# nvlong21/Lightweight-face-detection-CenterNet

Hardware: AMD Instinct MI355X
Metric: images/sec at 640x640 batch inference (higher is better)
Workload: dtype bf16; 1 GPU; BASELINE configs[1]: batch=64 640x640 bf16 on 1 MI355X per rank, forward + top-100 peak decode; synthetic uint8 images resident in HBM, calibrated synthetic weights (seed 0); 2 context(s) per GPU, batch k on context k mod 2; batch_per_gpu=64, global_batch=64, topk=100, parallelism=dp1, contexts_per_gpu=2, input_buffers=4

## Files before the change

### lightweight-face-detection-centernet_amd/csrc/cf_mbconv3.hip

```cpp
#include "cf_exp.h"
#include "cf_common.h"
#include "cf_kernels.h"
#include "cf_mx.h"
#include <cstdlib>

namespace cf {

template <int KS, int JX, int TOH, int TOW, int NW, bool ALDS = true>
struct Mx {
    static constexpr int HC = 32;
    static constexpr int IH = TOH + KS - 1, IWQ = TOW / 4 + 1, IWP = IWQ * 4;
    static constexpr int NQD = IH * IWQ, NIB = (NQD + 7) / 8, IPX = NQD * 4;
    static constexpr int CP = HC * 8 + 16;
    static constexpr int EBYTES = NIB * 8 * CP;
    static constexpr int NOQ = TOH * (TOW / 4), NSET = (NOQ + 15) / 16;
    static constexpr int WXB = JX * 1024;
    static constexpr int NSTEP = KS * 2;
    static constexpr int ATB = 2 * NSTEP * 512;
    static constexpr int LDS = EBYTES + WXB + (ALDS ? ATB : 0);
    static_assert(TOW % 4 == 0 && KS <= 5, "x-quads; two k-steps cover 4 + KS - 1 <= 8 inputs");
};

template <int KS, int JX, int TOH, int TOW, int NW, bool ALDS>
__global__ __launch_bounds__(NW * 64) void expdw_mx_kernel(MbParams p) {
    typedef Mx<KS, JX, TOH, TOW, NW, ALDS> G;
    constexpr int IWQ = G::IWQ, IWP = G::IWP, IPX = G::IPX, NIB = G::NIB, CP = G::CP, NSET = G::NSET, WXB = G::WXB;
    extern __shared__ __attribute__((aligned(16))) char smem[];
    char* E = smem;
    char* Wst = smem + G::EBYTES;

    const int tid = threadIdx.x, lane = tid & 63;
    const int wave = __builtin_amdgcn_readfirstlane(tid >> 6);
    const int pl = lane & 31, h = lane >> 5;
    const int tiles_x = (p.Wout + TOW - 1) / TOW;
    const int tyi = blockIdx.x / tiles_x, txi = blockIdx.x - tyi * tiles_x;
    const int ox0 = txi * TOW, oy0 = tyi * TOH, b = blockIdx.z;
    const int grp = blockIdx.y;

    {
        const char* srcx = (const char*)p.wexp + (size_t)grp * WXB;
        for (int c = wave; c < WXB / 1024; c += NW)
            __builtin_amdgcn_global_load_lds((const __attribute__((address_space(1))) void*)(srcx + c * 1024 + lane * 16),
                                             (__attribute__((address_space(3))) void*)(Wst + c * 1024), 16, 0, 0);
    }
    asm volatile("" ::: "memory");
    char* Ats = Wst + WXB;
    u32x2 A[ALDS ? 1 : 2][ALDS ? 1 : KS][2];
    if constexpr (ALDS) {
        const char* srca = (const char*)p.wdw + (size_t)grp * G::ATB;
        for (int c = wave; c < G::ATB / 1024; c += NW)
            __builtin_amdgcn_global_load_lds((const __attribute__((address_space(1))) void*)(srca + c * 1024 + lane * 16),
                                             (__attribute__((address_space(3))) void*)(Ats + c * 1024), 16, 0, 0);
    } else {
        const u32x2* at = reinterpret_cast<const u32x2*>(p.wdw) + (size_t)grp * (2 * KS * 2) * 64 + lane;
#pragma unroll
        for (int q = 0; q < 2; ++q)
#pragma unroll
            for (int ky = 0; ky < KS; ++ky)
#pragma unroll
                for (int ks = 0; ks < 2; ++ks) A[q][ky][ks] = at[((q * KS + ky) * 2 + ks) * 64];
    }
    asm volatile("" ::: "memory");
    const char* xbase = (const char*)p.x + (size_t)b * p.Hin * p.Win * p.Cin * 2;
    const unsigned rowbytes = (unsigned)p.Cin * 2;
    auto load_x = [&](int ib, u32x4* xf) -> bool {
        const int ip = ib * 32 + pl;
        const int ipc = ip < IPX ? ip : IPX - 1;
        const int iy = ipc / IWP, ix = ipc - iy * IWP;
        const int gy = oy0 - p.pad_lo + iy, gx = ox0 - p.pad_lo + ix;
        const int cy = min(max(gy, 0), p.Hin - 1), cx = min(max(gx, 0), p.Win - 1);
        if (p.xblock) {
            const char* xb = (const char*)p.x + blk_off(((size_t)b * p.Hin + cy) * p.Win + cx, p.Cin / 8, h * JX);
#pragma unroll
            for (int j = 0; j < JX; ++j) xf[j] = ld16(xb + j * 512);
        } else {
            const unsigned off = ((unsigned)cy * (unsigned)p.Win + (unsigned)cx) * rowbytes + (unsigned)(h * JX * 16);
#pragma unroll
            for (int j = 0; j < JX; ++j) xf[j] = ld16(xbase + off + j * 16);
        }
        return ip < IPX && (unsigned)gy < (unsigned)p.Hin && (unsigned)gx < (unsigned)p.Win;
    };
    const bool last_in = (h * JX + JX - 1) * 8 < p.Cin;
    auto mask_x = [&](u32x4* xf, bool valid) {
#pragma unroll
        for (int j = 0; j < JX; ++j) {
            const bool vj = j == JX - 1 ? (valid && last_in) : valid;
            xf[j].x = vj ? xf[j].x : 0u; xf[j].y = vj ? xf[j].y : 0u; xf[j].z = vj ? xf[j].z : 0u; xf[j].w = vj ? xf[j].w : 0u;
        }
    };
#ifdef CF_ABLATION
    const int abl = p.nw;
#else
    constexpr int abl = 0;
#endif
    u32x4 xa[JX];
    bool va = false;
    if (wave < NIB) va = load_x(wave, xa);
    static_assert(NIB >= NW, "every wave issues the X loads the wait below keeps in flight");
    cf_sync_lds_dma_keep<(ALDS ? 0 : 2 * KS * 2) + JX>();
    mask_x(xa, va);

    for (int ib = wave; ib < NIB; ib += NW) {
        u32x4 xn[JX];
        const bool more = ib + NW < NIB;
        bool vn = false;
        if (more) { if (abl & 8) { for (int j = 0; j < JX; ++j) xn[j] = xa[j]; vn = va; } else vn = load_x(ib + NW, xn); }
        f32x16 a;
#pragma unroll
        for (int r = 0; r < 16; ++r) a[r] = 0.0f;
        const char* wb = Wst + lane * 16;
#pragma unroll
        for (int j = 0; j < JX; ++j) {
            const u32x4 wv = ld16(wb + j * 1024);
            a = __builtin_amdgcn_mfma_f32_32x32x16_bf16(__builtin_bit_cast(mfma_bf16x8, xa[j]),
                                                        __builtin_bit_cast(mfma_bf16x8, wv), a, 0, 0, 0);
        }
        char* ecell = E + (unsigned)(ib * 8 + h) * (unsigned)CP + pl * 8;
#pragma unroll
        for (int t = 0; t < 4; ++t) {
            f32x2 u0, u1; u0.x = a[4 * t]; u0.y = a[4 * t + 1]; u1.x = a[4 * t + 2]; u1.y = a[4 * t + 3];
            f32x2 y0 = u0, y1 = u1;
            if (!(abl & 4)) { y0 = swish2_pre(u0); y1 = swish2_pre(u1); }
            u32x2 d;
            d.x = __builtin_bit_cast(uint32_t, __builtin_amdgcn_cvt_pkrtz(y0.x, y0.y));
            d.y = __builtin_bit_cast(uint32_t, __builtin_amdgcn_cvt_pkrtz(y1.x, y1.y));
            *reinterpret_cast<u32x2*>(ecell + 2 * t * CP) = d;
        }
        if (more) {
#pragma unroll
            for (int j = 0; j < JX; ++j) xa[j] = xn[j];
            mask_x(xa, vn);
        }
    }
    __syncthreads();

    static constexpr SetMap<TOH, TOW, IWQ> kSets{};
    const int kg = lane >> 4;
    for (int set = wave; set < NSET; set += NW) {
        const uint32_t e = kSets.v[set * 16 + (lane & 15)];
        const int oy = (e >> 6) & 0x1ff, oxq = e & 63;
        const bool live = (e & 0x8000u) == 0;
        f32x4 acc[8];
        const char* bb = E + (unsigned)(oy * IWQ + oxq) * (unsigned)CP + kg * 64;
        if (abl & 1) {
#pragma unroll
            for (int g = 0; g < 8; ++g) acc[g] = f32x4{(float)oy, (float)oxq, (float)g, 1.0f};
        } else {
        if constexpr (ALDS) mx_depthwise_lds<KS, IWQ, CP>(bb, Ats + lane * 8, acc);
        else mx_depthwise<KS, IWQ, CP>(bb, reinterpret_cast<const u32x2 (*)[KS][2]>(A), acc);
        }
        if (!(abl & 2))
#pragma unroll
        for (int g = 0; g < 8; ++g)
#pragma unroll
            for (int i = 0; i < 4; i += 2) {
                f32x2 u; u.x = acc[g][i]; u.y = acc[g][i + 1];
                const f32x2 y = swish2_pre(u) * kNegLn23;
                acc[g][i] = y.x; acc[g][i + 1] = y.y;
            }
        const int gy = oy0 + oy, gx0 = ox0 + 4 * oxq;
        if (!live || gy >= p.Hout || ((abl & 16) && acc[0][0] != 123.0f)) continue;
        const size_t opix0 = ((size_t)b * p.Hout + gy) * p.Wout + gx0;
        const int chunk = grp * 4 + kg;
#pragma unroll
        for (int i = 0; i < 4; ++i) {
            if (gx0 + i >= p.Wout) break;
            u32x4 o;
            o.x = packb(acc[0][i], acc[1][i]); o.y = packb(acc[2][i], acc[3][i]);
            o.z = packb(acc[4][i], acc[5][i]); o.w = packb(acc[6][i], acc[7][i]);
            const size_t opix = opix0 + i;
            if (abl & 32) {
                const size_t region = (((size_t)b * gridDim.x + blockIdx.x) * gridDim.y + grp) * (size_t)(TOH * TOW * 64);
                st16((char*)p.y + region + ((size_t)((set * 4 + i) * 1024 + lane * 16)) % (size_t)(TOH * TOW * 64), o);
                continue;
            }
            st16((char*)p.y + (p.yblock ? blk_off(opix, p.hid / 8, chunk) : (opix * p.hid + (size_t)chunk * 8) * 2), o);
        }
    }
}

#include CF_EXP_INC(cf_mbconv3_0)

template <int KS, int JX, int NMB, int TOH, int TOW, int NW, bool TAIL16, bool ALDS = false>
struct Fx {
    static constexpr int IH = TOH + KS - 1, IWQ = TOW / 4 + 1, IWP = IWQ * 4;
    static constexpr int NQD = IH * IWQ, NIB = (NQD + 7) / 8, IPX = NQD * 4, MAXI = (NIB + NW - 1) / NW;
    static constexpr int CP8 = 32 * 8 + 16, CP4 = 16 * 8 + 16;
    static constexpr int EBYTES = NIB * 8 * CP8;
    static constexpr int NOQ = TOH * (TOW / 4), NSET = (NOQ + 15) / 16, SPW = NSET / NW;
    static constexpr int WXB = JX * 1024;
    static constexpr int ATB = 2 * KS * 2 * 512;
    static constexpr int LDS = EBYTES + 2 * WXB + (ALDS ? ATB : 0);
    static_assert(NSET % NW == 0, "every wave owns SPW whole sets (project accumulators live in registers)");
    static_assert(TOW % 4 == 0 && KS <= 5 && (NMB == 2 || NMB == 4 || NMB == 6), "geometry");
    static_assert(!TAIL16 || JX <= 2, "16-channel round: one 16x16x32 expand MFMA, Cin <= 32");
};

template <int KS, int JX, int NMB, bool RESID, int TOH, int TOW, int NW, bool TAIL16, bool XRELOAD, bool ALDS, bool SB = false>
__global__ __launch_bounds__(NW * 64) void mbconv_mx_kernel(MbParams p) {
    typedef Fx<KS, JX, NMB, TOH, TOW, NW, TAIL16, ALDS> G;
    constexpr int IWQ = G::IWQ, IWP = G::IWP, IPX = G::IPX, NIB = G::NIB, MAXI = G::MAXI, CP8 = G::CP8, CP4 = G::CP4;
    constexpr int SPW = G::SPW, WXB = G::WXB;
    extern __shared__ __attribute__((aligned(16))) char smem[];
    char* E = smem;
    char* Wst = smem + G::EBYTES;
    char* Ats = Wst + 2 * G::WXB;

    const int tid = threadIdx.x, lane = tid & 63;
    const int wave = __builtin_amdgcn_readfirstlane(tid >> 6);
    const int pl = lane & 31, h = lane >> 5, kg = lane >> 4;
    const int ox0 = blockIdx.x * TOW, oy0 = blockIdx.y * TOH, b = blockIdx.z;
    const int nq = p.nq;
#ifdef CF_ABLATION
    const int abl = p.nw;
#else
    constexpr int abl = 0;
#endif

    const char* xbase = (const char*)p.x + (size_t)b * p.Hin * p.Win * p.Cin * 2;
    const unsigned rowbytes = (unsigned)p.Cin * 2;

    auto stage_weights = [&](int q) {
        char* dst = Wst + (q & 1) * WXB;
        const char* srcx = (const char*)p.wexp + (size_t)q * WXB;
        for (int c = wave; c < WXB / 1024; c += NW)
            __builtin_amdgcn_global_load_lds((const __attribute__((address_space(1))) void*)(srcx + c * 1024 + lane * 16),
                                             (__attribute__((address_space(3))) void*)(dst + c * 1024), 16, 0, 0);
    };

    u32x4 xf[MAXI][JX];
    auto load_x = [&]() {
#pragma unroll
    for (int t = 0; t < MAXI; ++t) {
        const int ib = wave + NW * t;
        const int ip = ib * 32 + pl;
        const int ipc = ip < IPX ? ip : IPX - 1;
        const int iy = ipc / IWP, ix = ipc - iy * IWP;
        const int gy = oy0 - p.pad_lo + iy, gx = ox0 - p.pad_lo + ix;
        const bool valid = ip < IPX && (unsigned)gy < (unsigned)p.Hin && (unsigned)gx < (unsigned)p.Win;
        const int cy = min(max(gy, 0), p.Hin - 1), cx = min(max(gx, 0), p.Win - 1);
        const unsigned off = ((unsigned)cy * (unsigned)p.Win + (unsigned)cx) * rowbytes + (unsigned)(h * JX * 16);
#pragma unroll
        for (int j = 0; j < JX; ++j) {
            const bool vj = valid && (h * JX + j) * 8 < p.Cin;
            const u32x4 v = ld16(xbase + off + j * 16);
            xf[t][j].x = vj ? v.x : 0u; xf[t][j].y = vj ? v.y : 0u;
            xf[t][j].z = vj ? v.z : 0u; xf[t][j].w = vj ? v.w : 0u;
        }
    }
    };
    if constexpr (!XRELOAD) load_x();

    static constexpr SetMap<TOH, TOW, IWQ> kSets{};
    unsigned qcell[SPW];
#pragma unroll
    for (int sw = 0; sw < SPW; ++sw) {
        const uint32_t e = kSets.v[(wave * SPW + sw) * 16 + (lane & 15)];
        qcell[sw] = ((e >> 6) & 0x1ff) * IWQ + (e & 63);
    }

    f32x4 pacc[SPW][4][NMB];
#pragma unroll
    for (int sw = 0; sw < SPW; ++sw)
#pragma unroll
        for (int i = 0; i < 4; ++i)
#pragma unroll
            for (int mb = 0; mb < NMB; ++mb) pacc[sw][i][mb] = f32x4{0.0f, 0.0f, 0.0f, 0.0f};

    stage_weights(0);
    asm volatile("" ::: "memory");
    for (int q = 0; q < nq; ++q) {
        const char* wx = Wst + (q & 1) * WXB;
        u32x2 A[ALDS ? 1 : 2][ALDS ? 1 : KS][2];
        if constexpr (!ALDS) {
            const u32x2* at = reinterpret_cast<const u32x2*>(p.wdw) + (size_t)q * (2 * KS * 2) * 64 + lane;
#pragma unroll
            for (int a = 0; a < 2; ++a)
#pragma unroll
                for (int ky = 0; ky < KS; ++ky)
#pragma unroll
                    for (int ks = 0; ks < 2; ++ks) A[a][ky][ks] = at[((a * KS + ky) * 2 + ks) * 64];
        }
        u32x4 wpc[NMB];
#pragma unroll
        for (int mb = 0; mb < NMB; ++mb) wpc[mb] = ld16((const char*)p.wproj + (((size_t)q * NMB + mb) * 64 + lane) * 16);
        if constexpr (XRELOAD) load_x();
        cf_sync_lds_dma_keep<(ALDS ? 0 : 2 * KS * 2) + NMB + (XRELOAD ? MAXI * JX : 0)>();
        if constexpr (ALDS) {
            const char* srca = (const char*)p.wdw + (size_t)q * G::ATB;
            for (int c = wave; c < G::ATB / 1024; c += NW)
                __builtin_amdgcn_global_load_lds((const __attribute__((address_space(1))) void*)(srca + c * 1024 + lane * 16),
                                                 (__attribute__((address_space(3))) void*)(Ats + c * 1024), 16, 0, 0);
        }
        const char* Atq = Ats;

#pragma unroll
        for (int t = 0; t < MAXI; ++t) {
            const int ib = wave + NW * t;
            if (ib >= NIB) break;
            f32x16 a;
#pragma unroll
            for (int r = 0; r < 16; ++r) a[r] = 0.0f;
#pragma unroll
            for (int j = 0; j < JX; ++j) {
                const u32x4 wv = ld16(wx + (j * 64 + lane) * 16);
                a = __builtin_amdgcn_mfma_f32_32x32x16_bf16(__builtin_bit_cast(mfma_bf16x8, xf[t][j]),
                                                            __builtin_bit_cast(mfma_bf16x8, wv), a, 0, 0, 0);
            }
            char* ecell = E + (unsigned)(ib * 8 + h) * (unsigned)CP8 + pl * 8;
#pragma unroll
            for (int tq = 0; tq < 4; ++tq) {
                f32x2 u0, u1; u0.x = a[4 * tq]; u0.y = a[4 * tq + 1]; u1.x = a[4 * tq + 2]; u1.y = a[4 * tq + 3];
                f32x2 y0 = u0, y1 = u1;
                if (!(abl & 4)) { y0 = swish2_pre(u0); y1 = swish2_pre(u1); }
                u32x2 d;
                d.x = __builtin_bit_cast(uint32_t, __builtin_amdgcn_cvt_pkrtz(y0.x, y0.y));
                d.y = __builtin_bit_cast(uint32_t, __builtin_amdgcn_cvt_pkrtz(y1.x, y1.y));
                *reinterpret_cast<u32x2*>(ecell + 2 * tq * CP8) = d;
            }
        }
        cf_sync_lds_dma();
        if (q + 1 < nq) stage_weights(q + 1);
        asm volatile("" ::: "memory");

#pragma unroll
        for (int sw = 0; sw < SPW; ++sw) {
            f32x4 acc[8];
            if (abl & 1) {
#pragma unroll
                for (int g = 0; g < 8; ++g) acc[g] = f32x4{(float)q, (float)g, 1.0f, 2.0f};
            } else {
            if constexpr (ALDS && SB) mx_depthwise_lds1<KS, IWQ, CP8>(E + qcell[sw] * (unsigned)CP8 + kg * 64, Atq + lane * 8, acc);
            else if constexpr (ALDS) mx_depthwise_lds<KS, IWQ, CP8>(E + qcell[sw] * (unsigned)CP8 + kg * 64, Atq + lane * 8, acc);
            else mx_depthwise<KS, IWQ, CP8>(E + qcell[sw] * (unsigned)CP8 + kg * 64, reinterpret_cast<const u32x2 (*)[KS][2]>(A), acc);
            }
            if (!(abl & 2))
#pragma unroll
            for (int g = 0; g < 8; ++g)
#pragma unroll
                for (int i = 0; i < 4; i += 2) {
                    f32x2 u; u.x = acc[g][i]; u.y = acc[g][i + 1];
                    const f32x2 y = swish2_pre(u);
                    acc[g][i] = y.x; acc[g][i + 1] = y.y;
                }
#pragma unroll
            for (int i = 0; i < 4; ++i) {
                u32x4 d;
                d.x = packb(acc[0][i], acc[1][i]); d.y = packb(acc[2][i], acc[3][i]);
                d.z = packb(acc[4][i], acc[5][i]); d.w = packb(acc[6][i], acc[7][i]);
                if (abl & 8) { pacc[sw][i][0][0] += __uint_as_float(d.x ^ d.y ^ d.z ^ d.w); continue; }
#pragma unroll
                for (int mb = 0; mb < NMB; ++mb)
                    pacc[sw][i][mb] = __builtin_amdgcn_mfma_f32_16x16x32_bf16(__builtin_bit_cast(mfma_bf16x8, wpc[mb]),
                                                                             __builtin_bit_cast(mfma_bf16x8, d), pacc[sw][i][mb], 0, 0, 0);
            }
        }
    }

    if constexpr (TAIL16) {
        typedef __attribute__((ext_vector_type(4))) __bf16 mfma_bf16x4;
        const u32x4 wv = ld16((const char*)p.wexp + (size_t)nq * WXB + lane * 16);
        u32x2 A4[KS][2];
        {
            const u32x2* at = reinterpret_cast<const u32x2*>(p.wdw) + (size_t)nq * (2 * KS * 2) * 64 + lane;
#pragma unroll
            for (int ky = 0; ky < KS; ++ky)
#pragma unroll
                for (int ks = 0; ks < 2; ++ks) A4[ky][ks] = at[(ky * 2 + ks) * 64];
        }
        u32x2 wp4[NMB];
#pragma unroll
        for (int mb = 0; mb < NMB; ++mb)
            wp4[mb] = *reinterpret_cast<const u32x2*>((const char*)p.wproj + (size_t)nq * NMB * 1024 + ((size_t)mb * 64 + lane) * 8);
        __syncthreads();
        for (int sb = wave; sb < NIB * 2; sb += NW) {
            const int ip = sb * 16 + (lane & 15), kc = lane >> 4;
            const int ipc = ip < IPX ? ip : IPX - 1;
            const int iy = ipc / IWP, ix = ipc - iy * IWP;
            const int gy = oy0 - p.pad_lo + iy, gx = ox0 - p.pad_lo + ix;
            const bool valid = ip < IPX && (unsigned)gy < (unsigned)p.Hin && (unsigned)gx < (unsigned)p.Win && kc * 8 < p.Cin;
            const int cy = min(max(gy, 0), p.Hin - 1), cx = min(max(gx, 0), p.Win - 1);
            u32x4 xv = ld16(xbase + ((unsigned)cy * (unsigned)p.Win + (unsigned)cx) * rowbytes + (unsigned)(min(kc * 8, p.Cin - 8) * 2));
            xv.x = valid ? xv.x : 0u; xv.y = valid ? xv.y : 0u; xv.z = valid ? xv.z : 0u; xv.w = valid ? xv.w : 0u;
            f32x4 a4 = {0.0f, 0.0f, 0.0f, 0.0f};
            a4 = __builtin_amdgcn_mfma_f32_16x16x32_bf16(__builtin_bit_cast(mfma_bf16x8, xv), __builtin_bit_cast(mfma_bf16x8, wv), a4, 0, 0, 0);
            f32x2 u0, u1; u0.x = a4[0]; u0.y = a4[1]; u1.x = a4[2]; u1.y = a4[3];
            const f32x2 y0 = swish2_pre(u0), y1 = swish2_pre(u1);
            u32x2 d;
            d.x = __builtin_bit_cast(uint32_t, __builtin_amdgcn_cvt_pkrtz(y0.x, y0.y));
            d.y = __builtin_bit_cast(uint32_t, __builtin_amdgcn_cvt_pkrtz(y1.x, y1.y));
            *reinterpret_cast<u32x2*>(E + (unsigned)(sb * 4 + kc) * (unsigned)CP4 + (lane & 15) * 8) = d;
        }
        __syncthreads();
#pragma unroll
        for (int sw = 0; sw < SPW; ++sw) {
            const char* bb = E + qcell[sw] * (unsigned)CP4 + kg * 32;
            f32x4 acc[4];
#pragma unroll
            for (int g = 0; g < 4; ++g) acc[g] = f32x4{0.0f, 0.0f, 0.0f, 0.0f};
#pragma unroll
            for (int st = 0; st < KS * 2; ++st) {
                const char* bs = bb + ((st >> 1) * IWQ + (st & 1)) * CP4;
// ... 646 lines not shown
```

### lightweight-face-detection-centernet_amd/csrc/cf_mx.h

```cpp
#pragma once
#include "cf_common.h"

namespace cf {

typedef __attribute__((ext_vector_type(8))) __bf16 mfma_bf16x8;
typedef __attribute__((ext_vector_type(4))) _Float16 mfma_f16x4;
static constexpr float kNegLog2e3 = -1.44269504088896341f, kNegLn23 = -0.69314718055994531f;

typedef __attribute__((ext_vector_type(2))) __bf16 bf16x2_v;
__device__ __forceinline__ uint32_t packb(float lo, float hi) {
    f32x2 v; v.x = lo; v.y = hi;
    return __builtin_bit_cast(uint32_t, __builtin_convertvector(v, bf16x2_v));
}
__device__ __forceinline__ u32x4 pack16b(const float* f) {
    u32x4 c; c.x = packb(f[0], f[1]); c.y = packb(f[2], f[3]); c.z = packb(f[4], f[5]); c.w = packb(f[6], f[7]); return c;
}

__device__ __forceinline__ f32x2 swish2_pre(f32x2 u) {
    f32x2 e; e.x = __builtin_amdgcn_exp2f(u.x); e.y = __builtin_amdgcn_exp2f(u.y);
    const f32x2 den = e + 1.0f;
    f32x2 r; r.x = __builtin_amdgcn_rcpf(den.x); r.y = __builtin_amdgcn_rcpf(den.y);
    return u * r;
}

static inline uint16_t host_f32_to_f16_3(float f) {
    uint32_t u; __builtin_memcpy(&u, &f, 4);
    const uint32_t sign = (u >> 16) & 0x8000u;
    const int32_t exp = (int32_t)((u >> 23) & 0xff) - 127 + 15;
    uint32_t man = u & 0x7fffffu;
    if (((u >> 23) & 0xff) == 0xff) return (uint16_t)(sign | 0x7c00u | (man ? 0x200u : 0));
    if (exp >= 31) return (uint16_t)(sign | 0x7bffu);
    if (exp <= 0) {
        if (exp < -10) return (uint16_t)sign;
        man |= 0x800000u;
        const int shift = 14 - exp;
        uint32_t half = man >> shift;
        const uint32_t rem = man & ((1u << shift) - 1), mid = 1u << (shift - 1);
        if (rem > mid || (rem == mid && (half & 1))) ++half;
        return (uint16_t)(sign | half);
    }
    uint32_t half = ((uint32_t)exp << 10) | (man >> 13);
    const uint32_t rem = man & 0x1fffu;
    if (rem > 0x1000u || (rem == 0x1000u && (half & 1))) ++half;
    if (half >= 0x7c00u) half = 0x7bffu;
    return (uint16_t)(sign | half);
}

template <int TOH, int TOW, int IWQ, int S = 1>
struct SetMap {
    static constexpr int OWQ = TOW / 4, NOQ = TOH * OWQ, NSET = (NOQ + 15) / 16, NSLOT = NSET * 16;
    static_assert(OWQ <= 64 && TOH <= 256, "entry packing");
    uint16_t v[NSLOT];
    constexpr SetMap() : v() {
        int bucket[16][NOQ] = {}; int cnt[16] = {}, used[16] = {};
        for (int r = 0; r < NOQ; ++r) { const int b = (S * (r / OWQ) * IWQ + (r % OWQ)) & 15; bucket[b][cnt[b]++] = r; }
        int slot[NSLOT] = {};
        for (int s = 0; s < NSET; ++s)
            for (int q = 0; q < 16; ++q) {
                const int b = ((q >> 2) + 4 * (q & 3)) & 15;
                slot[s * 16 + q] = used[b] < cnt[b] ? bucket[b][used[b]++] : -1;
            }
        for (int b = 0; b < 16; ++b)
            while (used[b] < cnt[b]) {
                int s = 0; while (slot[s] >= 0) ++s;
                slot[s] = bucket[b][used[b]++];
            }
        for (int s = 0; s < NSLOT; ++s) {
            const int r = slot[s] >= 0 ? slot[s] : 0;
            v[s] = (uint16_t)((slot[s] < 0 ? 0x8000 : 0) | ((r / OWQ) << 6) | (r % OWQ));
        }
    }
};

#define CF_MX_MFMA(ACC, AV, BV, ABID) ACC = __builtin_amdgcn_mfma_f32_4x4x4f16(AV, BV, ACC, 2, ABID, 0)

template <int KS, int IWQ, int CP>
__device__ __forceinline__ void mx_depthwise(const char* bb, const u32x2 (*A)[KS][2], f32x4* acc) {
    constexpr int NSTEP = KS * 2;
#pragma unroll
    for (int g = 0; g < 8; ++g) acc[g] = f32x4{0.0f, 0.0f, 0.0f, 0.0f};
    u32x4 bq[2][4];
#pragma unroll
    for (int g2 = 0; g2 < 4; ++g2) bq[0][g2] = ld16(bb + g2 * 16);
#pragma unroll
    for (int st = 0; st < NSTEP; ++st) {
        if (st + 1 < NSTEP) {
            const int ky = (st + 1) >> 1, ks = (st + 1) & 1;
#pragma unroll
            for (int g2 = 0; g2 < 4; ++g2) bq[(st + 1) & 1][g2] = ld16(bb + (ky * IWQ + ks) * CP + g2 * 16);
        }
        __builtin_amdgcn_sched_barrier(0);
#pragma unroll
        for (int g = 0; g < 8; ++g) {
            const mfma_f16x4 av = __builtin_bit_cast(mfma_f16x4, A[g >> 2][st >> 1][st & 1]);
            u32x2 b2;
            b2.x = (g & 1) ? bq[st & 1][g >> 1].z : bq[st & 1][g >> 1].x;
            b2.y = (g & 1) ? bq[st & 1][g >> 1].w : bq[st & 1][g >> 1].y;
            const mfma_f16x4 bv = __builtin_bit_cast(mfma_f16x4, b2);
            switch (g & 3) {
                case 0: CF_MX_MFMA(acc[g], av, bv, 0); break;
                case 1: CF_MX_MFMA(acc[g], av, bv, 1); break;
                case 2: CF_MX_MFMA(acc[g], av, bv, 2); break;
                default: CF_MX_MFMA(acc[g], av, bv, 3); break;
            }
        }
        __builtin_amdgcn_sched_barrier(0);
    }
}

template <int KS, int IWQ, int CP>
__device__ __forceinline__ void mx_depthwise_lds(const char* bb, const char* at , f32x4* acc) {
    constexpr int NSTEP = KS * 2;
#pragma unroll
    for (int g = 0; g < 8; ++g) acc[g] = f32x4{0.0f, 0.0f, 0.0f, 0.0f};
    u32x4 bq[2][4];
    u32x2 aq[2][2];
#pragma unroll
    for (int g2 = 0; g2 < 4; ++g2) bq[0][g2] = ld16(bb + g2 * 16);
    aq[0][0] = *reinterpret_cast<const u32x2*>(at);
    aq[0][1] = *reinterpret_cast<const u32x2*>(at + NSTEP * 512);
#pragma unroll
    for (int st = 0; st < NSTEP; ++st) {
        if (st + 1 < NSTEP) {
            const int ky = (st + 1) >> 1, ks = (st + 1) & 1;
#pragma unroll
            for (int g2 = 0; g2 < 4; ++g2) bq[(st + 1) & 1][g2] = ld16(bb + (ky * IWQ + ks) * CP + g2 * 16);
            aq[(st + 1) & 1][0] = *reinterpret_cast<const u32x2*>(at + (st + 1) * 512);
            aq[(st + 1) & 1][1] = *reinterpret_cast<const u32x2*>(at + (NSTEP + st + 1) * 512);
        }
        __builtin_amdgcn_sched_barrier(0);
#pragma unroll
        for (int g = 0; g < 8; ++g) {
            const mfma_f16x4 av = __builtin_bit_cast(mfma_f16x4, aq[st & 1][g >> 2]);
            u32x2 b2;
            b2.x = (g & 1) ? bq[st & 1][g >> 1].z : bq[st & 1][g >> 1].x;
            b2.y = (g & 1) ? bq[st & 1][g >> 1].w : bq[st & 1][g >> 1].y;
            const mfma_f16x4 bv = __builtin_bit_cast(mfma_f16x4, b2);
            switch (g & 3) {
                case 0: CF_MX_MFMA(acc[g], av, bv, 0); break;
                case 1: CF_MX_MFMA(acc[g], av, bv, 1); break;
                case 2: CF_MX_MFMA(acc[g], av, bv, 2); break;
                default: CF_MX_MFMA(acc[g], av, bv, 3); break;
            }
        }
        __builtin_amdgcn_sched_barrier(0);
    }
}

template <int KS, int IWQ, int CP>
__device__ __forceinline__ void mx_depthwise_lds1(const char* bb, const char* at, f32x4* acc) {
    constexpr int NSTEP = KS * 2;
#pragma unroll
    for (int g = 0; g < 8; ++g) acc[g] = f32x4{0.0f, 0.0f, 0.0f, 0.0f};
#pragma unroll
    for (int st = 0; st < NSTEP; ++st) {
        const int ky = st >> 1, ks = st & 1;
// ... 87 lines not shown
```

### lightweight-face-detection-centernet_amd/csrc/cf_stem0.hip

```cpp
#include <type_traits>
#include "cf_common.h"
#include "cf_kernels.h"
#include "cf_mx.h"
#include <vector>
#include "centerface_hip.h"

namespace cf {

typedef __attribute__((ext_vector_type(8))) __bf16 mfma_bf16x8;

static inline int slot_channel(int nb, int i) {
    int h = (i >> 2) & 1;
    int r = (i & 3) + 4 * (i >> 3);
    return nb * 32 + h * 16 + r;
}

constexpr int S0_TOH = 16, S0_TOW = 16;
constexpr int S0_NT = (S0_TOH * S0_TOW / 32) * 64;
constexpr int S0_IH = S0_TOH + 2, S0_IW = S0_TOW + 2, S0_IPX = S0_IH * S0_IW;
constexpr int S0_PH = 2 * S0_IH + 1, S0_PW = 2 * S0_IW + 1;
constexpr int S0_PROW = S0_PW * 3 + 1;

void stem0_lut(float* lut ) {
    const float mean[3] = {0.408f, 0.447f, 0.470f};
// ... 465 lines not shown
                if (decltype(lastb)::value && (tt & 1) + 4 * (tt >> 1) >= VP) continue;
                f32x2 x2; x2.x = a[2 * tt]; x2.y = a[2 * tt + 1];
                const f32x2 y2 = s0_swish2_prescaled(x2);
                *reinterpret_cast<uint32_t*>(ecol + ((tt & 1) + 4 * (tt >> 1)) * S0P_PITCH) =
                    __builtin_bit_cast(uint32_t, __builtin_amdgcn_cvt_pkrtz(y2.x, y2.y));
            }
        };
        if (VP < 16 && t == (S0P_NIB - 1) / S0P_NW && ib == S0P_NIB - 1) activate(std::true_type{});
        else activate(std::false_type{});
    }
    __syncthreads();

    const int par = wave >> 1;
    auto tile_pixel = [](int u, int& oy, int& ox) {
        const int pr = u >> 7, r = u & 127;
        oy = r >> 3; ox = 2 * (r & 7) + pr;
    };
    int dy, dx; tile_pixel((wave * 2 + h) * 32 + pl, dy, dx);
    const char* eb0 = E + (unsigned)((dy * S0_IW + (dx - par)) / 2) * (unsigned)S0P_PITCH;
    const S0_AS4 s0_u32x8* wtab = (const S0_AS4 s0_u32x8*)p.wdw;

    auto dw_chunk = [&](int c) -> u32x4 {
        float a8[8];
        const S0_AS4 s0_u32x8* wq = wtab + ((par * 4 + c) * 3) * 2;
        const char* eb = eb0 + c * 32;
#pragma unroll
        for (int ky = 0; ky < 3; ++ky)
#pragma unroll
            for (int t = 0; t < 2; ++t) {
                const s0_u32x8 wv = wq[ky * 2 + t];
                const char* et = eb + (ky * (S0_IW / 2) + t) * S0P_PITCH;
                const u32x4 e0 = ld16(et), e1 = ld16(et + 16);
                if (ky == 0 && t == 0) { dot8_first(a8, wv, e0, e1); continue; }
                s0_dot2c(a8[0], wv[0], e0.x); s0_dot2c(a8[1], wv[1], e0.y);
                s0_dot2c(a8[2], wv[2], e0.z); s0_dot2c(a8[3], wv[3], e0.w);
                s0_dot2c(a8[4], wv[4], e1.x); s0_dot2c(a8[5], wv[5], e1.y);
                s0_dot2c(a8[6], wv[6], e1.z); s0_dot2c(a8[7], wv[7], e1.w);
            }
#pragma unroll
        for (int i = 0; i < 8; i += 2) {
            f32x2 u; u.x = a8[i]; u.y = a8[i + 1];
            const f32x2 yv = s0_swish2_prescaled(u);
            a8[i] = yv.x; a8[i + 1] = yv.y;
        }
        return pack16<T>(a8);
    };

    f32x16 acc[2];
#pragma unroll
    for (int k = 0; k < 2; ++k)
#pragma unroll
        for (int r = 0; r < 16; ++r) acc[k][r] = 0.0f;
#pragma unroll
    for (int j = 0; j < 2; ++j) {
        const u32x4 wpc = ld16((const char*)p.wproj + ((size_t)j * 64 + lane) * 16);
        const u32x4 dA = dw_chunk(j), dB = dw_chunk(2 + j);
        u32x4 x0, x1;
        {
            auto s0 = __builtin_amdgcn_permlane32_swap(dA.x, dB.x, false, false); x0.x = s0[0]; x1.x = s0[1];
            auto s1 = __builtin_amdgcn_permlane32_swap(dA.y, dB.y, false, false); x0.y = s1[0]; x1.y = s1[1];
            auto s2 = __builtin_amdgcn_permlane32_swap(dA.z, dB.z, false, false); x0.z = s2[0]; x1.z = s2[1];
            auto s3 = __builtin_amdgcn_permlane32_swap(dA.w, dB.w, false, false); x0.w = s3[0]; x1.w = s3[1];
        }
        acc[0] = __builtin_amdgcn_mfma_f32_32x32x16_bf16(__builtin_bit_cast(mfma_bf16x8, wpc), __builtin_bit_cast(mfma_bf16x8, x0), acc[0], 0, 0, 0);
        acc[1] = __builtin_amdgcn_mfma_f32_32x32x16_bf16(__builtin_bit_cast(mfma_bf16x8, wpc), __builtin_bit_cast(mfma_bf16x8, x1), acc[1], 0, 0, 0);
    }
    if (h != 0) return;
#pragma unroll
    for (int k = 0; k < 2; ++k) {
        int oy, ox; tile_pixel((wave * 2 + k) * 32 + pl, oy, ox);
        const int gy = oy0 + oy, gx = ox0 + ox;
        if (gy >= Ho || gx >= Wo) continue;
        T* out = (T*)p.y + (((size_t)b * Ho + gy) * Wo + gx) * 16;
#pragma unroll
        for (int g = 0; g < 2; ++g) {
            float v[8];
#pragma unroll
            for (int e = 0; e < 8; ++e) v[e] = acc[k][g * 8 + e];
            st16(out + g * 8, pack16<T>(v));
        }
    }
}

constexpr int S0M_IWQ = S0_TOW / 4 + 1, S0M_IWP = 4 * S0M_IWQ;
constexpr int S0M_IPX = S0_IH * S0M_IWP, S0M_NIB = (S0_IH * S0M_IWQ + 7) / 8, S0M_CP = 32 * 8 + 16;
size_t stem0mx_wdw_dwords() { return 2 * 3 * 2 * 64 * 2; }
void stem0mx_pack(const float* ws, const float* wd, const float* wp, void* wstem_out, uint32_t* wdw_out, void* wproj_out) {
    std::vector<uint32_t> scratch(stem0px_wdw_dwords());
    std::vector<char> pscratch(stem0_proj_bytes(1));
    stem0px_pack(ws, wd, wp, wstem_out, scratch.data(), pscratch.data());
    mx_pack_taps(1, 3, wd, wdw_out);
    __builtin_memset(wproj_out, 0, stem0_proj_bytes(1));
    for (int lane = 0; lane < 64; ++lane) {
        const int co = lane & 15, kc = lane >> 4;
        uint16_t* dst = (uint16_t*)((char*)wproj_out + (size_t)lane * 16);
        for (int e = 0; e < 8; ++e) dst[e] = host_f32_to_bf16(kS0NegLn2 * wp[co * 32 + kc * 8 + e]);
    }
}

template <int FMT>
__global__ __launch_bounds__(S0P_NT) void stem0_mx_kernel(Stem0Params p) {
    typedef bf16_t T;
    __shared__ __attribute__((aligned(16))) char E[S0M_NIB * 8 * S0M_CP];
    static_assert(S0_PH * S0P_PROW * 2 <= S0M_NIB * 8 * S0M_CP, "patch must fit under the tile");
    T* Xs = reinterpret_cast<T*>(E);

    const int tid = threadIdx.x, lane = tid & 63;
    const int wave = __builtin_amdgcn_readfirstlane(tid >> 6);
    const int pl = lane & 31, h = lane >> 5;
    const int Ho = p.H >> 1, Wo = p.W >> 1;
    unsigned tbx = blockIdx.x, tby = blockIdx.y, tbz = blockIdx.z;
    if (p.kind & STEM0_XCD) xcd_tile_order(tbx, tby, tbz);
    const int ox0 = tbx * S0_TOW, oy0 = tby * S0_TOH, b = tbz;

    const int iy0 = 2 * (oy0 - 1), ix0 = 2 * (ox0 - 1);
    if constexpr (FMT == CF_IN_U8_HWC_BGR) {
        constexpr int ND = S0P_ND, RG = S0P_NT / ND, NITD = (S0_PH + RG - 1) / RG;
        const int d = tid % ND, rg = tid / ND;
        const bool tact = rg < RG;
        const int boff = ix0 * 3 - 2 + 4 * d;
        const bool din = tact && boff >= 0 && boff + 4 <= p.W * 3;
        const int cboff = min(max(boff, 0), p.W * 3 - 4);
        float sc[4], sh[4]; bool bok[4];
#pragma unroll
        for (int i = 0; i < 4; ++i) {
            const int e = 4 * d - 2 + i;
            bok[i] = din && e >= 0 && e < S0_PW * 3;
            const int ci = (e + 3) % 3;
            sc[i] = ci == 0 ? 1.0f / (255.0f * 0.289f) : ci == 1 ? 1.0f / (255.0f * 0.274f) : 1.0f / (255.0f * 0.278f);
            sh[i] = ci == 0 ? -0.408f / 0.289f : ci == 1 ? -0.447f / 0.274f : -0.470f / 0.278f;
        }
        uint32_t v[NITD];
#pragma unroll
        for (int it = 0; it < NITD; ++it) {
            const int cy = min(max(iy0 + rg + it * RG, 0), p.H - 1);
            v[it] = *reinterpret_cast<const uint32_t*>((const uint8_t*)p.x + ((size_t)b * p.H + cy) * p.W * 3 + cboff);
        }
        const bool interior = iy0 >= 0 && iy0 + S0_PH <= p.H && ix0 * 3 - 2 >= 0 && ix0 * 3 - 2 + 4 * ND <= p.W * 3;
        auto convert = [&](auto inside) {
#pragma unroll
            for (int it = 0; it < NITD; ++it) {
                const int r = rg + it * RG, iy = iy0 + r;
                const bool rowok = (unsigned)iy < (unsigned)p.H;
                float f[4];
#pragma unroll
                for (int i = 0; i < 4; ++i) {
                    const float u = (float)((v[it] >> (8 * i)) & 0xffu);
                    const float nv = fmaf(u, sc[i], sh[i]);
                    f[i] = (decltype(inside)::value || (rowok && bok[i])) ? nv : 0.0f;
                }
                if (tact && r < S0_PH) {
                    u32x2 o; o.x = pack_bf16x2(f[0], f[1]); o.y = pack_bf16x2(f[2], f[3]);
                    *reinterpret_cast<u32x2*>(reinterpret_cast<char*>(Xs) + r * (S0P_PROW * 2) + d * 8) = o;
                }
            }
        };
        if (interior) convert(std::true_type{}); else convert(std::false_type{});
    } else {
        constexpr int ECOLS = S0_PW * 3, RSTEP = S0P_NT / ECOLS, NIT = (S0_PH + RSTEP - 1) / RSTEP;
        const int e = tid % ECOLS, r0 = tid / ECOLS;
        const bool tact = r0 < RSTEP;
        const int col = e / 3, ci = e - col * 3;
        const int ix = ix0 + col;
        const bool xok = tact && (unsigned)ix < (unsigned)p.W;
        const int cx = min(max(ix, 0), p.W - 1);
        float v[NIT];
#pragma unroll
        for (int it = 0; it < NIT; ++it) {
            const int r = r0 + it * RSTEP;
            const int iy = iy0 + r;
            const bool ok = xok && r < S0_PH && (unsigned)iy < (unsigned)p.H;
            const int cy = min(max(iy, 0), p.H - 1);
            const float f = ((const float*)p.x)[(((size_t)b * 3 + ci) * p.H + cy) * p.W + cx];
            v[it] = ok ? f : 0.0f;
        }
#pragma unroll
        for (int it = 0; it < NIT; ++it) {
            const int r = r0 + it * RSTEP;
            if (tact && r < S0_PH) Xs[r * S0P_PROW + 2 + e] = (T)(pack_bf16x2(v[it], 0.0f) & 0xffffu);
        }
    }
    __syncthreads();

    u32x4 ws[2];
#pragma unroll
    for (int c = 0; c < 2; ++c) ws[c] = ld16((const char*)p.wstem + ((size_t)c * 64 + lane) * 16);
    u32x2 A[2][3][2];
    {
        const u32x2* at = reinterpret_cast<const u32x2*>(p.wdw) + lane;
#pragma unroll
        for (int q = 0; q < 2; ++q)
#pragma unroll
            for (int ky = 0; ky < 3; ++ky)
#pragma unroll
                for (int ks = 0; ks < 2; ++ks) A[q][ky][ks] = at[((q * 3 + ky) * 2 + ks) * 64];
    }
    constexpr int MAXB = (S0M_NIB + S0P_NW - 1) / S0P_NW;
    u32x4 xg[MAXB][2];
    const bool halo_inside = oy0 >= 1 && oy0 + S0_TOH + 1 <= Ho && ox0 >= 1 && ox0 + S0_TOW + 1 <= Wo;
    auto gather = [&](auto inside) {
#pragma unroll
    for (int t = 0; t < MAXB; ++t) {
        const int ib = wave + S0P_NW * t;
        const int ip = ib * 32 + pl;
        const int ipc = ip < S0M_IPX ? ip : S0M_IPX - 1;
        const int ty = ipc / S0M_IWP, txq = ipc - ty * S0M_IWP, tx = txq < S0_IW ? txq : S0_IW - 1;
        const int y = oy0 - 1 + ty, x = ox0 - 1 + tx;
        const bool inmap = decltype(inside)::value || (ip < S0M_IPX && (unsigned)y < (unsigned)Ho && (unsigned)x < (unsigned)Wo);
        const char* xp = reinterpret_cast<const char*>(Xs) + ((2 * ty) * S0P_PROW + (2 * tx) * 3 + 2) * 2;
#pragma unroll
        for (int c = 0; c < 2; ++c) {
            uint32_t w4[4];
#pragma unroll
            for (int i = 0; i < 4; ++i) {
                const int off = c == 0 ? h * (S0P_PROW * 2) + 4 * i
                                       : (h == 0 ? 2 * (S0P_PROW * 2) + 4 * i : 16 + (i < 2 ? i : 2) * (S0P_PROW * 2));
                const uint32_t v = *reinterpret_cast<const uint32_t*>(xp + off);
                w4[i] = inmap ? v : 0u;
            }
            xg[t][c].x = w4[0]; xg[t][c].y = w4[1]; xg[t][c].z = w4[2]; xg[t][c].w = w4[3];
        }
    }
    };
    if (halo_inside) gather(std::true_type{}); else gather(std::false_type{});
    __syncthreads();
#pragma unroll
    for (int t = 0; t < MAXB; ++t) {
        const int ib = wave + S0P_NW * t;
        if (ib >= S0M_NIB) break;
        f32x16 a;
#pragma unroll
        for (int r = 0; r < 16; ++r) a[r] = 0.0f;
#pragma unroll
        for (int c = 0; c < 2; ++c)
            a = __builtin_amdgcn_mfma_f32_32x32x16_bf16(__builtin_bit_cast(mfma_bf16x8, xg[t][c]),
                                                        __builtin_bit_cast(mfma_bf16x8, ws[c]), a, 0, 0, 0);
        char* ecell = E + (unsigned)(ib * 8 + h) * (unsigned)S0M_CP + pl * 8;
#pragma unroll
        for (int tq = 0; tq < 4; ++tq) {
            f32x2 u0, u1; u0.x = a[4 * tq]; u0.y = a[4 * tq + 1]; u1.x = a[4 * tq + 2]; u1.y = a[4 * tq + 3];
            const f32x2 y0 = swish2_pre(u0), y1 = swish2_pre(u1);
            u32x2 d;
            d.x = __builtin_bit_cast(uint32_t, __builtin_amdgcn_cvt_pkrtz(y0.x, y0.y));
            d.y = __builtin_bit_cast(uint32_t, __builtin_amdgcn_cvt_pkrtz(y1.x, y1.y));
            *reinterpret_cast<u32x2*>(ecell + 2 * tq * S0M_CP) = d;
        }
    }
    __syncthreads();

    static constexpr SetMap<S0_TOH, S0_TOW, S0M_IWQ> kSets{};
    const uint32_t se = kSets.v[wave * 16 + (lane & 15)];
    const int soy = (se >> 6) & 0x1ff, soxq = se & 63, kg = lane >> 4;
    f32x4 acc[8];
    mx_depthwise<3, S0M_IWQ, S0M_CP>(E + (unsigned)(soy * S0M_IWQ + soxq) * (unsigned)S0M_CP + kg * 64,
                                      reinterpret_cast<const u32x2 (*)[3][2]>(A), acc);
#pragma unroll
    for (int g = 0; g < 8; ++g)
#pragma unroll
        for (int i = 0; i < 4; i += 2) {
            f32x2 u; u.x = acc[g][i]; u.y = acc[g][i + 1];
            const f32x2 yv = swish2_pre(u);
            acc[g][i] = yv.x; acc[g][i + 1] = yv.y;
        }
    const u32x4 wpc = ld16((const char*)p.wproj + (size_t)lane * 16);
    const int gy = oy0 + soy, gx0 = ox0 + 4 * soxq;
#pragma unroll
    for (int i = 0; i < 4; ++i) {
        u32x4 d;
        d.x = packb(acc[0][i], acc[1][i]); d.y = packb(acc[2][i], acc[3][i]);
        d.z = packb(acc[4][i], acc[5][i]); d.w = packb(acc[6][i], acc[7][i]);
        f32x4 o = {0.0f, 0.0f, 0.0f, 0.0f};
        o = __builtin_amdgcn_mfma_f32_16x16x32_bf16(__builtin_bit_cast(mfma_bf16x8, wpc), __builtin_bit_cast(mfma_bf16x8, d), o, 0, 0, 0);
        if (gy < Ho && gx0 + i < Wo) {
            u32x2 ov; ov.x = packb(o[0], o[1]); ov.y = packb(o[2], o[3]);
            *reinterpret_cast<u32x2*>((T*)p.y + (((size_t)b * Ho + gy) * Wo + gx0 + i) * 16 + kg * 4) = ov;
        }
    }
}

hipError_t launch_stem0(hipStream_t s, int dtype, const Stem0Params& p) {
    if (p.B <= 0) return hipSuccess;
    const int Ho = p.H / 2, Wo = p.W / 2;
    if (p.kind & STEM0_MX) {
        if (dtype != 1) return hipErrorInvalidValue;
        dim3 grid((Wo + S0_TOW - 1) / S0_TOW, (Ho + S0_TOH - 1) / S0_TOH, p.B), blk(S0P_NT);
        set_kernel_tag("void cf::stem0_mx_kernel<%d>(cf::Stem0Params)", p.in_format);
        if (p.in_format == CF_IN_U8_HWC_BGR) hipLaunchKernelGGL((stem0_mx_kernel<CF_IN_U8_HWC_BGR>), grid, blk, 0, s, p);
        else hipLaunchKernelGGL((stem0_mx_kernel<CF_IN_F32_NCHW>), grid, blk, 0, s, p);
        return hipGetLastError();
    }
    if (p.kind & STEM0_PX) {
        if (dtype != 1) return hipErrorInvalidValue;
        dim3 grid((Wo + S0_TOW - 1) / S0_TOW, (Ho + S0_TOH - 1) / S0_TOH, p.B), blk(S0P_NT);
        set_kernel_tag("void cf::stem0_px_kernel<%d>(cf::Stem0Params)", p.in_format);
        if (p.in_format == CF_IN_U8_HWC_BGR) hipLaunchKernelGGL((stem0_px_kernel<CF_IN_U8_HWC_BGR>), grid, blk, 0, s, p);
        else hipLaunchKernelGGL((stem0_px_kernel<CF_IN_F32_NCHW>), grid, blk, 0, s, p);
        return hipGetLastError();
    }
    dim3 grid((Wo + S0_TOW - 1) / S0_TOW, (Ho + S0_TOH - 1) / S0_TOH, p.B), blk(S0_NT);
    set_kernel_tag("void cf::stem0_kernel<%s, %d>(cf::Stem0Params)", dtype == 0 ? "float" : dtype == 2 ? "sp32_t" : "unsigned short", p.in_format);
    if (dtype == 0) {
        if (p.in_format == CF_IN_U8_HWC_BGR) hipLaunchKernelGGL((stem0_kernel<float, CF_IN_U8_HWC_BGR>), grid, blk, 0, s, p);
        else hipLaunchKernelGGL((stem0_kernel<float, CF_IN_F32_NCHW>), grid, blk, 0, s, p);
    } else if (dtype == 2) {
        if (p.in_format == CF_IN_U8_HWC_BGR) hipLaunchKernelGGL((stem0_kernel<sp32_t, CF_IN_U8_HWC_BGR>), grid, blk, 0, s, p);
        else hipLaunchKernelGGL((stem0_kernel<sp32_t, CF_IN_F32_NCHW>), grid, blk, 0, s, p);
    } else {
        if (p.in_format == CF_IN_U8_HWC_BGR) hipLaunchKernelGGL((stem0_kernel<bf16_t, CF_IN_U8_HWC_BGR>), grid, blk, 0, s, p);
        else hipLaunchKernelGGL((stem0_kernel<bf16_t, CF_IN_F32_NCHW>), grid, blk, 0, s, p);
    }
    return hipGetLastError();
}

#ifdef CF_X5_TIMING
}
extern "C" int cf_debug_stem_stamps(unsigned long long* out6, int reset) {
    static unsigned long long host[204800 * 8];
    if (hipMemcpyFromSymbol(host, HIP_SYMBOL(cf::g_s0_buf), sizeof host) != hipSuccess) return -1;
    if (out6) { for (int k = 0; k < 6; ++k) out6[k] = 0; for (size_t w = 0; w < 204800; ++w) for (int k = 0; k < 6; ++k) out6[k] += host[w * 8 + k]; }
    if (reset) { static unsigned long long z[204800 * 8]; if (hipMemcpyToSymbol(HIP_SYMBOL(cf::g_s0_buf), z, sizeof z) != hipSuccess) return -1; }
    return 0;
}
namespace cf {
#endif
}
```

Before: 54100 images/s.

## Reorder halo pixel quads so tail column pairs skip redundant swish and stores

Adds a TailOrder slot map that sends the full-width x-quads of each row pair first and the last (partial) quad column afterwards. The expand-conv output stage then stores cells by closed-form address. For tail quads it skips the swish and conversion of the unused upper half and writes zeros there. This applies to the stem0 fused kernel and to KS=3 fused MBConv kernels with an even halo height, and replaces the linear ip/IWP div-mod index with a compile-time table formula. The intent is to cut wasted activation math on halo padding columns and drop an integer division. The price is more intricate index logic and branchy store paths.

```diff
diff --git a/lightweight-face-detection-centernet_amd/csrc/cf_mbconv3.hip b/lightweight-face-detection-centernet_amd/csrc/cf_mbconv3.hip
--- a/lightweight-face-detection-centernet_amd/csrc/cf_mbconv3.hip
+++ b/lightweight-face-detection-centernet_amd/csrc/cf_mbconv3.hip
@@ -11,6 +11,7 @@
     static constexpr int HC = 32;
     static constexpr int IH = TOH + KS - 1, IWQ = TOW / 4 + 1, IWP = IWQ * 4;
     static constexpr int NQD = IH * IWQ, NIB = (NQD + 7) / 8, IPX = NQD * 4;
+    static constexpr bool TQ = false;
     static constexpr int CP = HC * 8 + 16;
     static constexpr int EBYTES = NIB * 8 * CP;
     static constexpr int NOQ = TOH * (TOW / 4), NSET = (NOQ + 15) / 16;
@@ -31,6 +32,8 @@
 
     const int tid = threadIdx.x, lane = tid & 63;
     const int wave = __builtin_amdgcn_readfirstlane(tid >> 6);
+    constexpr bool TQ = G::TQ;
+    if constexpr (TQ) __builtin_assume(wave >= 0 && wave < NW);
     const int pl = lane & 31, h = lane >> 5;
     const int tiles_x = (p.Wout + TOW - 1) / TOW;
     const int tyi = blockIdx.x / tiles_x, txi = blockIdx.x - tyi * tiles_x;
@@ -65,8 +68,14 @@
     const unsigned rowbytes = (unsigned)p.Cin * 2;
     auto load_x = [&](int ib, u32x4* xf) -> bool {
         const int ip = ib * 32 + pl;
-        const int ipc = ip < IPX ? ip : IPX - 1;
-        const int iy = ipc / IWP, ix = ipc - iy * IWP;
+        int iy, ix;
+        if constexpr (TQ) {
+            const uint32_t rq = TailOrder<TQ ? G::IH : 2, IWQ>::row_xq(min(ip >> 2, G::NQD - 1));
+            iy = rq >> 8; ix = 4 * (rq & 255) + (pl & 3);
+        } else {
+            const int ipc = ip < IPX ? ip : IPX - 1;
+            iy = ipc / IWP; ix = ipc - iy * IWP;
+        }
         const int gy = oy0 - p.pad_lo + iy, gx = ox0 - p.pad_lo + ix;
         const int cy = min(max(gy, 0), p.Hin - 1), cx = min(max(gx, 0), p.Win - 1);
         if (p.xblock) {
@@ -115,17 +124,7 @@
             a = __builtin_amdgcn_mfma_f32_32x32x16_bf16(__builtin_bit_cast(mfma_bf16x8, xa[j]),
                                                         __builtin_bit_cast(mfma_bf16x8, wv), a, 0, 0, 0);
         }
-        char* ecell = E + (unsigned)(ib * 8 + h) * (unsigned)CP + pl * 8;
-#pragma unroll
-        for (int t = 0; t < 4; ++t) {
-            f32x2 u0, u1; u0.x = a[4 * t]; u0.y = a[4 * t + 1]; u1.x = a[4 * t + 2]; u1.y = a[4 * t + 3];
-            f32x2 y0 = u0, y1 = u1;
-            if (!(abl & 4)) { y0 = swish2_pre(u0); y1 = swish2_pre(u1); }
-            u32x2 d;
-            d.x = __builtin_bit_cast(uint32_t, __builtin_amdgcn_cvt_pkrtz(y0.x, y0.y));
-            d.y = __builtin_bit_cast(uint32_t, __builtin_amdgcn_cvt_pkrtz(y1.x, y1.y));
-            *reinterpret_cast<u32x2*>(ecell + 2 * t * CP) = d;
-        }
+        mx_store_cells<TQ, G::IH, IWQ, CP>(a, E, ib, h, pl, !(abl & 4));
         if (more) {
 #pragma unroll
             for (int j = 0; j < JX; ++j) xa[j] = xn[j];
@@ -185,6 +184,7 @@
 struct Fx {
     static constexpr int IH = TOH + KS - 1, IWQ = TOW / 4 + 1, IWP = IWQ * 4;
     static constexpr int NQD = IH * IWQ, NIB = (NQD + 7) / 8, IPX = NQD * 4, MAXI = (NIB + NW - 1) / NW;
+    static constexpr bool TQ = KS == 3 && IH % 2 == 0;
     static constexpr int CP8 = 32 * 8 + 16, CP4 = 16 * 8 + 16;
     static constexpr int EBYTES = NIB * 8 * CP8;
     static constexpr int NOQ = TOH * (TOW / 4), NSET = (NOQ + 15) / 16, SPW = NSET / NW;
@@ -208,6 +208,8 @@
 
     const int tid = threadIdx.x, lane = tid & 63;
     const int wave = __builtin_amdgcn_readfirstlane(tid >> 6);
+    constexpr bool TQ = G::TQ;
+    if constexpr (TQ) __builtin_assume(wave >= 0 && wave < NW);
     const int pl = lane & 31, h = lane >> 5, kg = lane >> 4;
     const int ox0 = blockIdx.x * TOW, oy0 = blockIdx.y * TOH, b = blockIdx.z;
     const int nq = p.nq;
@@ -234,8 +236,14 @@
     for (int t = 0; t < MAXI; ++t) {
         const int ib = wave + NW * t;
         const int ip = ib * 32 + pl;
-        const int ipc = ip < IPX ? ip : IPX - 1;
-        const int iy = ipc / IWP, ix = ipc - iy * IWP;
+        int iy, ix;
+        if constexpr (TQ) {
+            const uint32_t rq = TailOrder<TQ ? G::IH : 2, IWQ>::row_xq(min(ip >> 2, G::NQD - 1));
+            iy = rq >> 8; ix = 4 * (rq & 255) + (pl & 3);
+        } else {
+            const int ipc = ip < IPX ? ip : IPX - 1;
+            iy = ipc / IWP; ix = ipc - iy * IWP;
+        }
         const int gy = oy0 - p.pad_lo + iy, gx = ox0 - p.pad_lo + ix;
         const bool valid = ip < IPX && (unsigned)gy < (unsigned)p.Hin && (unsigned)gx < (unsigned)p.Win;
         const int cy = min(max(gy, 0), p.Hin - 1), cx = min(max(gx, 0), p.Win - 1);
@@ -307,17 +315,7 @@
                 a = __builtin_amdgcn_mfma_f32_32x32x16_bf16(__builtin_bit_cast(mfma_bf16x8, xf[t][j]),
                                                             __builtin_bit_cast(mfma_bf16x8, wv), a, 0, 0, 0);
             }
-            char* ecell = E + (unsigned)(ib * 8 + h) * (unsigned)CP8 + pl * 8;
-#pragma unroll
-            for (int tq = 0; tq < 4; ++tq) {
-                f32x2 u0, u1; u0.x = a[4 * tq]; u0.y = a[4 * tq + 1]; u1.x = a[4 * tq + 2]; u1.y = a[4 * tq + 3];
-                f32x2 y0 = u0, y1 = u1;
-                if (!(abl & 4)) { y0 = swish2_pre(u0); y1 = swish2_pre(u1); }
-                u32x2 d;
-                d.x = __builtin_bit_cast(uint32_t, __builtin_amdgcn_cvt_pkrtz(y0.x, y0.y));
-                d.y = __builtin_bit_cast(uint32_t, __builtin_amdgcn_cvt_pkrtz(y1.x, y1.y));
-                *reinterpret_cast<u32x2*>(ecell + 2 * tq * CP8) = d;
-            }
+            mx_store_cells<TQ, G::IH, IWQ, CP8>(a, E, ib, h, pl, !(abl & 4));
         }
         cf_sync_lds_dma();
         if (q + 1 < nq) stage_weights(q + 1);
diff --git a/lightweight-face-detection-centernet_amd/csrc/cf_mx.h b/lightweight-face-detection-centernet_amd/csrc/cf_mx.h
--- a/lightweight-face-detection-centernet_amd/csrc/cf_mx.h
+++ b/lightweight-face-detection-centernet_amd/csrc/cf_mx.h
@@ -1,4 +1,5 @@
 #pragma once
+#include <type_traits>
 #include "cf_common.h"
 
 namespace cf {
@@ -72,6 +73,70 @@
     }
 };
 
+template <int IH, int IWQ>
+struct TailOrder {
+    static_assert(IH % 2 == 0, "pairs of halo rows");
+    static constexpr int W4 = IWQ - 1, NFP = IH / 2 * W4, NQD = IH * IWQ, NPR = NQD / 2;
+    uint16_t v[NQD];
+    static constexpr int row_xq(int s) {
+        const int pr = s >> 1, h = s & 1;
+        return pr < NFP ? ((2 * (pr / W4) + h) << 8) | (pr % W4) : ((2 * (pr - NFP) + h) << 8) | W4;
+    }
+    constexpr TailOrder() : v() {
+        for (int s = 0; s < NQD; ++s) v[s] = (uint16_t)row_xq(s);
+    }
+    static constexpr int pair_cell(int pr) { return pr < NFP ? 2 * (pr / W4) * IWQ + pr % W4 : 2 * (pr - NFP) * IWQ + W4; }
+    constexpr bool consistent() const {
+        bool seen[NQD] = {};
+        for (int s = 0; s < NQD; ++s) {
+            const int c = (v[s] >> 8) * IWQ + (v[s] & 255);
+            if (v[s] != row_xq(s) || c != pair_cell(s >> 1) + (s & 1) * IWQ || c >= NQD || seen[c]) return false;
+            seen[c] = true;
+        }
+        return true;
+    }
+};
+
+template <bool TQ, int IH, int IWQ, int CP>
+__device__ __forceinline__ void mx_store_cells(const f32x16& a, char* E, int ib, int h, int pl, bool act = true) {
+    auto half_quad = [&](int r) -> uint32_t {
+        f32x2 u; u.x = a[r]; u.y = a[r + 1];
+        const f32x2 y = act ? swish2_pre(u) : u;
+        return __builtin_bit_cast(uint32_t, __builtin_amdgcn_cvt_pkrtz(y.x, y.y));
+    };
+    if constexpr (TQ) {
+        typedef TailOrder<IH, IWQ> Q;
+        static constexpr Q kOrder{};
+        static_assert(kOrder.consistent(), "cell address closed form disagrees with the slot table");
+        char* ecell = E + (unsigned)(h * IWQ) * (unsigned)CP + pl * 8;
+        auto quad = [&](int tq, auto kind) {
+            const int pr = ib * 4 + tq;
+            const bool tail = decltype(kind)::value == 2 ? pr >= Q::NFP : decltype(kind)::value == 1;
+            u32x2 d; d.x = half_quad(4 * tq);
+            if (tail) d.y = 0u; else d.y = half_quad(4 * tq + 2);
+            const unsigned cell = tail ? (unsigned)(2 * (pr - Q::NFP) * IWQ + Q::W4) : (unsigned)(2 * (pr / Q::W4) * IWQ + pr % Q::W4);
+            *reinterpret_cast<u32x2*>(ecell + cell * (unsigned)CP) = d;
+        };
+        if (ib * 4 + 3 < Q::NFP) {
+#pragma unroll
+            for (int tq = 0; tq < 4; ++tq) quad(tq, std::integral_constant<int, 0>{});
+        } else if (Q::NFP % 4 == 0 || ib * 4 >= Q::NFP) {
+#pragma unroll
+            for (int tq = 0; tq < 4; ++tq) { if (ib * 4 + tq >= Q::NPR) break; quad(tq, std::integral_constant<int, 1>{}); }
+        } else {
+#pragma unroll
+            for (int tq = 0; tq < 4; ++tq) { if (ib * 4 + tq >= Q::NPR) break; quad(tq, std::integral_constant<int, 2>{}); }
+        }
+    } else {
+        char* ecell = E + (unsigned)(ib * 8 + h) * (unsigned)CP + pl * 8;
+#pragma unroll
+        for (int tq = 0; tq < 4; ++tq) {
+            u32x2 d; d.x = half_quad(4 * tq); d.y = half_quad(4 * tq + 2);
+            *reinterpret_cast<u32x2*>(ecell + 2 * tq * CP) = d;
+        }
+    }
+}
+
 #define CF_MX_MFMA(ACC, AV, BV, ABID) ACC = __builtin_amdgcn_mfma_f32_4x4x4f16(AV, BV, ACC, 2, ABID, 0)
 
 template <int KS, int IWQ, int CP>
diff --git a/lightweight-face-detection-centernet_amd/csrc/cf_stem0.hip b/lightweight-face-detection-centernet_amd/csrc/cf_stem0.hip
--- a/lightweight-face-detection-centernet_amd/csrc/cf_stem0.hip
+++ b/lightweight-face-detection-centernet_amd/csrc/cf_stem0.hip
@@ -571,8 +571,8 @@
     }
 }
 
-constexpr int S0M_IWQ = S0_TOW / 4 + 1, S0M_IWP = 4 * S0M_IWQ;
-constexpr int S0M_IPX = S0_IH * S0M_IWP, S0M_NIB = (S0_IH * S0M_IWQ + 7) / 8, S0M_CP = 32 * 8 + 16;
+constexpr int S0M_IWQ = S0_TOW / 4 + 1;
+constexpr int S0M_NQD = S0_IH * S0M_IWQ, S0M_NIB = (S0M_NQD + 7) / 8, S0M_CP = 32 * 8 + 16;
 size_t stem0mx_wdw_dwords() { return 2 * 3 * 2 * 64 * 2; }
 void stem0mx_pack(const float* ws, const float* wd, const float* wp, void* wstem_out, uint32_t* wdw_out, void* wproj_out) {
     std::vector<uint32_t> scratch(stem0px_wdw_dwords());
@@ -596,6 +596,7 @@
 
     const int tid = threadIdx.x, lane = tid & 63;
     const int wave = __builtin_amdgcn_readfirstlane(tid >> 6);
+    __builtin_assume(wave >= 0 && wave < S0P_NW);
     const int pl = lane & 31, h = lane >> 5;
     const int Ho = p.H >> 1, Wo = p.W >> 1;
     unsigned tbx = blockIdx.x, tby = blockIdx.y, tbz = blockIdx.z;
@@ -691,11 +692,11 @@
 #pragma unroll
     for (int t = 0; t < MAXB; ++t) {
         const int ib = wave + S0P_NW * t;
-        const int ip = ib * 32 + pl;
-        const int ipc = ip < S0M_IPX ? ip : S0M_IPX - 1;
-        const int ty = ipc / S0M_IWP, txq = ipc - ty * S0M_IWP, tx = txq < S0_IW ? txq : S0_IW - 1;
+        const int slot = ib * 8 + (pl >> 2);
+        const uint32_t rq = TailOrder<S0_IH, S0M_IWQ>::row_xq(slot < S0M_NQD ? slot : S0M_NQD - 1);
+        const int ty = rq >> 8, txq = 4 * (rq & 255) + (pl & 3), tx = txq < S0_IW ? txq : S0_IW - 1;
         const int y = oy0 - 1 + ty, x = ox0 - 1 + tx;
-        const bool inmap = decltype(inside)::value || (ip < S0M_IPX && (unsigned)y < (unsigned)Ho && (unsigned)x < (unsigned)Wo);
+        const bool inmap = decltype(inside)::value || (slot < S0M_NQD && (unsigned)y < (unsigned)Ho && (unsigned)x < (unsigned)Wo);
         const char* xp = reinterpret_cast<const char*>(Xs) + ((2 * ty) * S0P_PROW + (2 * tx) * 3 + 2) * 2;
 #pragma unroll
         for (int c = 0; c < 2; ++c) {
@@ -724,16 +725,7 @@
         for (int c = 0; c < 2; ++c)
             a = __builtin_amdgcn_mfma_f32_32x32x16_bf16(__builtin_bit_cast(mfma_bf16x8, xg[t][c]),
                                                         __builtin_bit_cast(mfma_bf16x8, ws[c]), a, 0, 0, 0);
-        char* ecell = E + (unsigned)(ib * 8 + h) * (unsigned)S0M_CP + pl * 8;
-#pragma unroll
-        for (int tq = 0; tq < 4; ++tq) {
-            f32x2 u0, u1; u0.x = a[4 * tq]; u0.y = a[4 * tq + 1]; u1.x = a[4 * tq + 2]; u1.y = a[4 * tq + 3];
-            const f32x2 y0 = swish2_pre(u0), y1 = swish2_pre(u1);
-            u32x2 d;
-            d.x = __builtin_bit_cast(uint32_t, __builtin_amdgcn_cvt_pkrtz(y0.x, y0.y));
-            d.y = __builtin_bit_cast(uint32_t, __builtin_amdgcn_cvt_pkrtz(y1.x, y1.y));
-            *reinterpret_cast<u32x2*>(ecell + 2 * tq * S0M_CP) = d;
-        }
+        mx_store_cells<true, S0_IH, S0M_IWQ, S0M_CP>(a, E, ib, h, pl);
     }
     __syncthreads();
 
```

Result: no change. 54200 images/s (median of 6 runs) (+0.2%).
